# HKPolyU-UAV/FLVIS

Hardware: AMD Instinct MI355X
Metric: frames/sec/node (640×480 stereo+IMU) + ATE vs CPU ref, EuRoC MH_05 (higher is better)
Workload: dtype u8/f32 LK+GFTT, f64 geometry+BA

## Files before the change

flvis_amd/csrc/lk_kernel.hip:

```cpp
#include "dev_common.hpp"
#include "img_kernels.hpp"

namespace flvis {

constexpr int LK_WIN = 31;
constexpr int LK_PS = 40;
constexpr int LK_PROWS = 34;
constexpr int LK_RM = 4;
constexpr int LK_RS = 52;
constexpr int LK_RROWS = 33 + 2 * LK_RM;
constexpr int LK_TC_HDR = 64;
constexpr int LK_TC_LVL = 64 * 24;

typedef short lk_s2 __attribute__((ext_vector_type(2)));
typedef __attribute__((address_space(1))) uint32_t lk_gu32;
typedef uint32_t lk_u4 __attribute__((ext_vector_type(4)));
__device__ __forceinline__ lk_s2 lk_as_s2(uint32_t v) { return __builtin_bit_cast(lk_s2, v); }

__device__ __forceinline__ bool lk_load_patch(const uint8_t* __restrict__ img, int w, int h, int pitch, int bx, int by, int X0, int Y0,
                                              int nrows, uint8_t* patch) {
  if (X0 >= -bx && Y0 >= -by && X0 + 39 < w + bx && Y0 + nrows <= h + by) {
    const lk_gu32* const base = (const lk_gu32*)(img + (ptrdiff_t)Y0 * pitch + (X0 & ~3));
    const int sh = X0 & 3;
    int r = (int)threadIdx.x / 9, k = (int)threadIdx.x - 9 * r;
    unsigned off = (unsigned)(r * pitch + 4 * k);
    static_assert(LK_PROWS * 9 <= 5 * 64, "five trips");
    const int n = nrows * 9;
    uint32_t lo[5], hi[5];
#pragma unroll
    for (int t = 0; t < 5; t++) {
      const bool on = (int)threadIdx.x + 64 * t < n;
      const unsigned o = on ? off : 0u;
      lo[t] = *(const lk_gu32*)((const __attribute__((address_space(1))) uint8_t*)base + o);
      hi[t] = *(const lk_gu32*)((const __attribute__((address_space(1))) uint8_t*)base + o + 4);
      k += 1;
      const bool wrap = k >= 9;
      k = wrap ? k - 9 : k;
      off += (unsigned)(7 * pitch + 4) + (wrap ? (unsigned)(pitch - 36) : 0u);
    }
#pragma unroll
    for (int t = 0; t < 5; t++) asm volatile("" : "+v"(lo[t]), "+v"(hi[t]));
    r = (int)threadIdx.x / 9;
    k = (int)threadIdx.x - 9 * r;
    unsigned dst = (unsigned)(r * LK_PS + 4 * k);
#pragma unroll
    for (int t = 0; t < 5; t++) {
      if ((int)threadIdx.x + 64 * t < n) *reinterpret_cast<uint32_t*>(patch + dst) = __builtin_amdgcn_alignbyte(hi[t], lo[t], sh);
      k += 1;
      const bool wrap = k >= 9;
      k = wrap ? k - 9 : k;
      dst += (unsigned)(7 * LK_PS + 4) + (wrap ? (unsigned)(LK_PS - 36) : 0u);
    }
    return false;
  }
  for (int i = threadIdx.x; i < nrows * 9; i += 64) {
    int r = i / 9, k = i - r * 9;
    int Y = Y0 + r, X = X0 + 4 * k;
    uint32_t v;
    if (Y >= 0 && Y < h && X >= 0 && X + 3 < w) {
      const uint8_t* row = img + (size_t)Y * pitch;
      int a = X & ~3, sh = X & 3;
      uint32_t lo = *reinterpret_cast<const uint32_t*>(row + a);
      uint32_t hi = sh ? *reinterpret_cast<const uint32_t*>(row + a + 4) : 0u;
      v = __builtin_amdgcn_alignbyte(hi, lo, sh);
    } else {
      const uint8_t* row = img + (size_t)reflect101c(Y, h) * pitch;
      uint32_t b0 = row[reflect101c(X, w)], b1 = row[reflect101c(X + 1, w)], b2 = row[reflect101c(X + 2, w)],
               b3 = row[reflect101c(X + 3, w)];
      v = b0 | (b1 << 8) | (b2 << 16) | (b3 << 24);
    }
    *reinterpret_cast<uint32_t*>(patch + r * LK_PS + 4 * k) = v;
  }
  return true;
}

__device__ __forceinline__ bool lk_load_region(const uint8_t* __restrict__ img, int w, int h, int pitch, int bx, int by, int X0, int Y0,
                                               uint8_t* region) {
  if (X0 >= -bx && Y0 >= -by && X0 + 51 < w + bx && Y0 + LK_RROWS <= h + by) {
    const __attribute__((address_space(1))) uint8_t* const base = (const __attribute__((address_space(1))) uint8_t*)(img + (ptrdiff_t)Y0 * pitch + X0);
    int r = (int)threadIdx.x / 13, k = (int)threadIdx.x - 13 * r;
    unsigned off = (unsigned)(r * pitch + 4 * k);
    static_assert(LK_RS == 52, "the region rows are contiguous in LDS: item i sits at byte 4 i");
    constexpr int N = LK_RROWS * 13, T = (N + 63) / 64;
    uint32_t v[T];
#pragma unroll
    for (int t = 0; t < T; t++) {
      const bool on = 64 * (t + 1) <= N || (int)threadIdx.x + 64 * t < N;
      v[t] = *(const lk_gu32*)(base + (on ? off : 0u));
      k += 12;
      const bool wrap = k >= 13;
      k = wrap ? k - 13 : k;
      off += (unsigned)(4 * pitch + 48) + (wrap ? (unsigned)(pitch - 52) : 0u);
    }
#pragma unroll
    for (int t = 0; t < T; t++) asm volatile("" : "+v"(v[t]));
#pragma unroll
    for (int t = 0; t < T; t++)
      if (64 * (t + 1) <= N || (int)threadIdx.x + 64 * t < N) *reinterpret_cast<uint32_t*>(region + 4 * ((int)threadIdx.x + 64 * t)) = v[t];
    return false;
  }
  for (int i = threadIdx.x; i < LK_RROWS * 13; i += 64) {
    int r = i / 13, k = i - r * 13;
    int Y = Y0 + r, X = X0 + 4 * k;
    uint32_t v;
    if (Y >= 0 && Y < h && X >= 0 && X + 3 < w) {
      v = *reinterpret_cast<const uint32_t*>(img + (size_t)Y * pitch + X);
    } else {
      const uint8_t* row = img + (size_t)reflect101c(Y, h) * pitch;
      uint32_t b0 = row[reflect101c(X, w)], b1 = row[reflect101c(X + 1, w)], b2 = row[reflect101c(X + 2, w)],
               b3 = row[reflect101c(X + 3, w)];
      v = b0 | (b1 << 8) | (b2 << 16) | (b3 << 24);
    }
    *reinterpret_cast<uint32_t*>(region + r * LK_RS + 4 * k) = v;
  }
  return true;
}

#define LK_PAIR(D, K)                                                                                              \
  ((((K)&3) == 3) ? __builtin_amdgcn_perm((D)[((K) >> 2) + 1], (D)[(K) >> 2], 0x0c040c03u)                         \
                  : __builtin_amdgcn_perm(0u, (D)[(K) >> 2], 0x0c000c00u | (uint32_t)((K)&3) | ((uint32_t)(((K)&3) + 1) << 16)))

__device__ __forceinline__ int lk_dot2_bias(lk_s2 a, lk_s2 b, int bias_uniform) {
  int r;
  asm("v_dot2_i32_i16 %0, %1, %2, %3" : "=v"(r) : "v"(a), "v"(b), "s"(bias_uniform));
  return r;
}
__device__ __forceinline__ void lk_wave_sum2_f32(int v1, int v2, float& f1, float& f2) {
  int a = v1 & 0xffff, b = v1 >> 16, c = v2 & 0xffff, d = v2 >> 16;
#define LK_STEP4(CTRL, RM)                                           \
  {                                                                  \
    const int ta = __builtin_amdgcn_update_dpp(0, a, CTRL, RM, 0xf, false); \
    const int tb = __builtin_amdgcn_update_dpp(0, b, CTRL, RM, 0xf, false); \
    const int tc = __builtin_amdgcn_update_dpp(0, c, CTRL, RM, 0xf, false); \
    const int td = __builtin_amdgcn_update_dpp(0, d, CTRL, RM, 0xf, false); \
    a += ta, b += tb, c += tc, d += td;                              \
  }
  LK_STEP4(0xB1, 0xf)
  LK_STEP4(0x4E, 0xf)
  LK_STEP4(0x141, 0xf)
  LK_STEP4(0x140, 0xf)
  LK_STEP4(0x142, 0xa)
  LK_STEP4(0x143, 0xc)
#undef LK_STEP4
  const float g1 = (float)__builtin_fma((double)b, 65536.0, (double)a), g2 = (float)__builtin_fma((double)d, 65536.0, (double)c);
  f1 = __builtin_bit_cast(float, __builtin_amdgcn_readlane(__builtin_bit_cast(int, g1), 63));
  f2 = __builtin_bit_cast(float, __builtin_amdgcn_readlane(__builtin_bit_cast(int, g2), 63));
}

__device__ __forceinline__ void lk_wave_sum3_wide(int v1, int v2, int v3, long long& s1, long long& s2, long long& s3) {
  int a = v1 & 0xffff, b = v1 >> 16, c = v2 & 0xffff, d = v2 >> 16, e = v3 & 0xffff, f = v3 >> 16;
#define LK_STEP6(CTRL, RM)                                                    \
  {                                                                           \
    const int ta = __builtin_amdgcn_update_dpp(0, a, CTRL, RM, 0xf, false);  \
    const int tb = __builtin_amdgcn_update_dpp(0, b, CTRL, RM, 0xf, false);  \
    const int tc = __builtin_amdgcn_update_dpp(0, c, CTRL, RM, 0xf, false);  \
    const int td = __builtin_amdgcn_update_dpp(0, d, CTRL, RM, 0xf, false);  \
    const int te = __builtin_amdgcn_update_dpp(0, e, CTRL, RM, 0xf, false);  \
    const int tf = __builtin_amdgcn_update_dpp(0, f, CTRL, RM, 0xf, false);  \
    a += ta, b += tb, c += tc, d += td, e += te, f += tf;                     \
  }
  LK_STEP6(0xB1, 0xf)
  LK_STEP6(0x4E, 0xf)
  LK_STEP6(0x141, 0xf)
  LK_STEP6(0x140, 0xf)
  LK_STEP6(0x142, 0xa)
  LK_STEP6(0x143, 0xc)
#undef LK_STEP6
  s1 = ((long long)__builtin_amdgcn_readlane(b, 63) << 16) + (long long)__builtin_amdgcn_readlane(a, 63);
  s2 = ((long long)__builtin_amdgcn_readlane(d, 63) << 16) + (long long)__builtin_amdgcn_readlane(c, 63);
  s3 = ((long long)__builtin_amdgcn_readlane(f, 63) << 16) + (long long)__builtin_amdgcn_readlane(e, 63);
}

template <bool INTERIOR>
__device__ __forceinline__ void lk_template(const uint8_t* patch, int lane, int ipx, int ipy, int W, int H, lk_s2 wT, lk_s2 wB,
                                            lk_s2 (&tI)[8], lk_s2 (&tX)[8], lk_s2 (&tY)[8], int& a11, int& a12, int& a22) {
  constexpr int W_BITS = 14;
  const int r = lane >> 1, c0 = (lane & 1) * 16;
  uint32_t d[3][5];
#pragma unroll
  for (int j = 0; j < 3; j++)
#pragma unroll
    for (int k = 0; k < 5; k++) d[j][k] = *reinterpret_cast<const uint32_t*>(patch + (r + j) * LK_PS + c0 + 4 * k);
  uint32_t bits = 0;
  if (!INTERIOR) {
    const int xs = ipx + c0, Y = ipy + r;
    int lo = -xs, hi = W - xs;
    lo = lo < 0 ? 0 : (lo > 18 ? 18 : lo);
    hi = hi < 0 ? 0 : (hi > 18 ? 18 : hi);
    bits = (Y >= 0 && Y < H && hi > lo) ? (((1u << hi) - 1u) & ~((1u << lo) - 1u)) : 0u;
  }
  lk_s2 DX[2][9], DY[2][9];
  {
    lk_s2 T0[10], T1[10];
#pragma unroll
    for (int j = 0; j < 10; j++) {
      const lk_s2 A = __builtin_bit_cast(lk_s2, LK_PAIR(d[0], 2 * j)), B = __builtin_bit_cast(lk_s2, LK_PAIR(d[1], 2 * j)),
                  Cc = __builtin_bit_cast(lk_s2, LK_PAIR(d[2], 2 * j));
      T0[j] = (A + Cc) * (short)3 + B * (short)10;
      T1[j] = Cc - A;
    }
    const int up2 = ((lane + 2) & 63) * 4;
#pragma unroll
    for (int j = 0; j < 9; j++) {
      DX[0][j] = T0[j + 1] - T0[j];
      const lk_s2 T1o = __builtin_bit_cast(lk_s2, __builtin_amdgcn_perm(__builtin_bit_cast(uint32_t, T1[j + 1]),
                                                                       __builtin_bit_cast(uint32_t, T1[j]), 0x05040302u));
      DY[0][j] = (T1[j + 1] + T1[j]) * (short)3 + T1o * (short)10;
      if (!INTERIOR) {
        const uint32_t m = ((bits >> (2 * j)) & 1u ? 0x0000ffffu : 0u) | ((bits >> (2 * j + 1)) & 1u ? 0xffff0000u : 0u);
        DX[0][j] = __builtin_bit_cast(lk_s2, __builtin_bit_cast(uint32_t, DX[0][j]) & m);
        DY[0][j] = __builtin_bit_cast(lk_s2, __builtin_bit_cast(uint32_t, DY[0][j]) & m);
      }
      DX[1][j] = __builtin_bit_cast(lk_s2, __builtin_amdgcn_ds_bpermute(up2, __builtin_bit_cast(int, DX[0][j])));
      DY[1][j] = __builtin_bit_cast(lk_s2, __builtin_amdgcn_ds_bpermute(up2, __builtin_bit_cast(int, DY[0][j])));
    }
  }
  if (r < LK_WIN) {
#pragma unroll
    for (int c2 = 0; c2 < 8; c2++) {
      int iv[2], ix[2], iy[2];
#pragma unroll
      for (int hh = 0; hh < 2; hh++) {
        const int c = 2 * c2 + hh;
        lk_s2 x0, x1, y0, y1;
        if (hh == 0) {
          x0 = DX[0][c2]; x1 = DX[1][c2]; y0 = DY[0][c2]; y1 = DY[1][c2];
        } else {
          x0 = __builtin_bit_cast(lk_s2, __builtin_amdgcn_perm(__builtin_bit_cast(uint32_t, DX[0][c2 + 1]), __builtin_bit_cast(uint32_t, DX[0][c2]), 0x05040302u));
          x1 = __builtin_bit_cast(lk_s2, __builtin_amdgcn_perm(__builtin_bit_cast(uint32_t, DX[1][c2 + 1]), __builtin_bit_cast(uint32_t, DX[1][c2]), 0x05040302u));
          y0 = __builtin_bit_cast(lk_s2, __builtin_amdgcn_perm(__builtin_bit_cast(uint32_t, DY[0][c2 + 1]), __builtin_bit_cast(uint32_t, DY[0][c2]), 0x05040302u));
          y1 = __builtin_bit_cast(lk_s2, __builtin_amdgcn_perm(__builtin_bit_cast(uint32_t, DY[1][c2 + 1]), __builtin_bit_cast(uint32_t, DY[1][c2]), 0x05040302u));
        }
        int ax = lk_dot2_bias(x0, wT, 1 << (W_BITS - 1)), ay = lk_dot2_bias(y0, wT, 1 << (W_BITS - 1));
        int ai = lk_dot2_bias(__builtin_bit_cast(lk_s2, LK_PAIR(d[1], c + 1)), wT, 1 << (W_BITS - 5 - 1));
        ax = __builtin_amdgcn_sdot2(x1, wB, ax, false);
        ay = __builtin_amdgcn_sdot2(y1, wB, ay, false);
        ai = __builtin_amdgcn_sdot2(__builtin_bit_cast(lk_s2, LK_PAIR(d[2], c + 1)), wB, ai, false);
        const bool on = c0 + c < LK_WIN;
        ix[hh] = on ? (ax >> W_BITS) : 0;
        iy[hh] = on ? (ay >> W_BITS) : 0;
        iv[hh] = on ? (ai >> (W_BITS - 5)) : 0;
      }
      tI[c2] = __builtin_bit_cast(lk_s2, __builtin_amdgcn_perm((uint32_t)iv[1], (uint32_t)iv[0], 0x05040100u));
      tX[c2] = __builtin_bit_cast(lk_s2, __builtin_amdgcn_perm((uint32_t)ix[1], (uint32_t)ix[0], 0x05040100u));
      tY[c2] = __builtin_bit_cast(lk_s2, __builtin_amdgcn_perm((uint32_t)iy[1], (uint32_t)iy[0], 0x05040100u));
      a11 = __builtin_amdgcn_sdot2(tX[c2], tX[c2], a11, false);
      a12 = __builtin_amdgcn_sdot2(tX[c2], tY[c2], a12, false);
      a22 = __builtin_amdgcn_sdot2(tY[c2], tY[c2], a22, false);
    }
  } else {
#pragma unroll
    for (int c = 0; c < 8; c++) {
      tI[c] = lk_s2{0, 0};
      tX[c] = lk_s2{0, 0};
      tY[c] = lk_s2{0, 0};
    }
  }
}

__device__ __forceinline__ bool lk_template_level(const uint8_t* img, int W, int H, int pitch, int bx, int by, int ipx, int ipy, int iw00,
                                                  int iw01, int iw10, int iw11, uint8_t* patch, int lane, lk_s2 (&tI)[8], lk_s2 (&tX)[8],
                                                  lk_s2 (&tY)[8], long long& iA11, long long& iA12, long long& iA22) {
  __syncthreads();
  const bool slow = lk_load_patch(img, W, H, pitch, bx, by, ipx - 1, ipy - 1, LK_PROWS, patch);
  __syncthreads();
  int a11 = 0, a12 = 0, a22 = 0;
  const bool interior = ipx >= 0 && ipx + 32 <= W - 1 && ipy >= 0 && ipy + 31 <= H - 1;
  const lk_s2 wT = lk_s2{(short)iw00, (short)iw01}, wB = lk_s2{(short)iw10, (short)iw11};
  if (interior)
    lk_template<true>(patch, lane, ipx, ipy, W, H, wT, wB, tI, tX, tY, a11, a12, a22);
  else
    lk_template<false>(patch, lane, ipx, ipy, W, H, wT, wB, tI, tX, tY, a11, a12, a22);
  lk_wave_sum3_wide(a11, a12, a22, iA11, iA12, iA22);
  return slow;
}
struct LKTmpl {
  uint32_t w[24];
  long long a11, a12, a22;
};
__device__ __noinline__ void lk_template_level_cold(const uint8_t* img, int W, int H, int pitch, int bx, int by, int ipx, int ipy, int iw00,
                                                    int iw01, int iw10, int iw11, uint8_t* patch, int lane, LKTmpl* out) {
  lk_s2 tI[8], tX[8], tY[8];
  long long a11, a12, a22;
  lk_template_level(img, W, H, pitch, bx, by, ipx, ipy, iw00, iw01, iw10, iw11, patch, lane, tI, tX, tY, a11, a12, a22);
#pragma unroll
  for (int k = 0; k < 8; k++) {
    out->w[k] = __builtin_bit_cast(uint32_t, tI[k]);
    out->w[8 + k] = __builtin_bit_cast(uint32_t, tX[k]);
    out->w[16 + k] = __builtin_bit_cast(uint32_t, tY[k]);
  }
  out->a11 = a11;
  out->a12 = a12;
  out->a22 = a22;
}

__device__ __forceinline__ void lk_tc_store_level(uint32_t* tc_ptr, int level, int lane, const lk_s2 (&tI)[8], const lk_s2 (&tX)[8],
                                                  const lk_s2 (&tY)[8], long long iA11, long long iA12, long long iA22) {
  lk_u4* dst = reinterpret_cast<lk_u4*>(tc_ptr + LK_TC_HDR + (size_t)level * LK_TC_LVL) + lane;
  uint32_t wI[8];
#pragma unroll
  for (int k = 0; k < 8; k++) wI[k] = __builtin_bit_cast(uint32_t, tI[k]);
  if (lane == 63) {
    wI[0] = (uint32_t)iA11; wI[1] = (uint32_t)((unsigned long long)iA11 >> 32);
    wI[2] = (uint32_t)iA12; wI[3] = (uint32_t)((unsigned long long)iA12 >> 32);
    wI[4] = (uint32_t)iA22; wI[5] = (uint32_t)((unsigned long long)iA22 >> 32);
  }
#pragma unroll
  for (int k = 0; k < 2; k++) {
    __builtin_nontemporal_store(lk_u4{wI[4 * k], wI[4 * k + 1], wI[4 * k + 2], wI[4 * k + 3]}, dst + 64 * k);
    __builtin_nontemporal_store(lk_u4{__builtin_bit_cast(uint32_t, tX[4 * k]), __builtin_bit_cast(uint32_t, tX[4 * k + 1]),
                                      __builtin_bit_cast(uint32_t, tX[4 * k + 2]), __builtin_bit_cast(uint32_t, tX[4 * k + 3])}, dst + 64 * (2 + k));
    __builtin_nontemporal_store(lk_u4{__builtin_bit_cast(uint32_t, tY[4 * k]), __builtin_bit_cast(uint32_t, tY[4 * k + 1]),
                                      __builtin_bit_cast(uint32_t, tY[4 * k + 2]), __builtin_bit_cast(uint32_t, tY[4 * k + 3])}, dst + 64 * (4 + k));
  }
}

__device__ __forceinline__ const uint8_t* lk_level_ptr(const PyrSel& P, int level, int s, int kc, const uint8_t* ind0) {
  const ImgSel& I = P.lvl[level];
  if (I.ind) return (level == 0 ? ind0 : *I.ind) + (size_t)s * P.stride[level];
  return I.b[I.cur ? (kc ^ I.flip) : 0] + (size_t)s * P.stride[level];
}

#ifndef FLVIS_LK_WAVES
#define FLVIS_LK_WAVES 4
#endif
#ifndef FLVIS_LK_WAVES_T
#define FLVIS_LK_WAVES_T 4
#endif
#ifdef FLVIS_LK_UTIL
__device__ unsigned long long g_lk_wt[3][8][32768][2];
#define LK_UTIL_BEGIN const unsigned long long lk_t0_ = wall_clock64(); const unsigned lk_widx_ = (blockIdx.y * gridDim.x + blockIdx.x) & 32767u;
#define LK_UTIL_END(ROLE)                                                              \
  if (threadIdx.x == 0) {                                                              \
    unsigned long long* u_ = g_lk_wt[(ROLE) % 3][prm.dbg_slot & 7][lk_widx_];          \
    u_[0] = lk_t0_;                                                                    \
    u_[1] = wall_clock64();                                                            \
  }
#else
#define LK_UTIL_BEGIN
#define LK_UTIL_END(ROLE)
#endif
template <int ROLE>
__device__ __forceinline__ void lk_track_body(const PyrSel& prev, const PyrSel& next, const float* __restrict__ prev_pts,
                                              float* __restrict__ next_pts, uint8_t* __restrict__ status,
                                              const int* __restrict__ count, int nmax, const LKParams& prm,
                                              const int* __restrict__ active) {
  int s = blockIdx.y, bx = blockIdx.x;
  {
    const int G = gridDim.x, N = G * gridDim.y;
    if ((N & 7) == 0) {
      const int L = bx + G * s;
      const int Lp = (L & 7) * (N >> 3) + (L >> 3);
      s = Lp / G;
      bx = Lp - s * G;
    }
  }
  if (active && !active[s]) return;
  int n = count[s];
  if (n > nmax) n = nmax;
  if (bx >= n) return;
  LK_UTIL_BEGIN
  __shared__ __attribute__((aligned(16))) uint8_t patch[LK_RROWS * LK_RS + 12];
  const int lane = threadIdx.x;
  int kc_prev = 0, kc_next = 0;
#pragma unroll
  for (int l = LK_MAX_LEVELS - 1; l >= 0; l--) {
    if (l <= prev.levels && prev.lvl[l].cur) kc_prev = prev.lvl[l].cur[s];
    if (l <= next.levels && next.lvl[l].cur) kc_next = next.lvl[l].cur[s];
  }
  const uint8_t* const ind_prev0 = prev.lvl[0].ind ? *prev.lvl[0].ind : nullptr;
  const uint8_t* const ind_next0 = next.lvl[0].ind ? *next.lvl[0].ind : nullptr;
  const int r = lane >> 1;
  const int c0 = (lane & 1) * 16;
  const int W_BITS = 14;
  double eps2 = prm.eps2;
  if (ROLE == 1) asm volatile("" : "+v"(eps2));
  const float FLT_SCALE = 1.f / (1 << 20);
  const float halfWin = (LK_WIN - 1) * 0.5f;

  for (int pb = bx; pb < n; pb += gridDim.x) {
    const int p = prm.order == 1 ? n - 1 - pb : pb;
    const size_t pi = ((size_t)s * nmax + p) * 2;
    const float ppx0 = prev_pts[pi], ppy0 = prev_pts[pi + 1];
    float nx = next_pts[pi], ny = next_pts[pi + 1];
    int st = 1;
    uint32_t* tc_ptr = nullptr;
    bool tc_store = false, tc_hit = false;
    uint32_t tc_mask = 0;
    if (ROLE == 2 && prm.tc_mode == 1) {
      if (p < prm.tc_cap) {
        tc_store = true;
        tc_ptr = prm.tc + ((size_t)s * prm.tc_cap + p) * prm.tc_stride;
      }
    } else if (ROLE == 1 && prm.tc_mode == 2) {
      const int code = __builtin_amdgcn_readfirstlane(prm.tc_slot[(size_t)s * nmax + p]);
      if (code >= 0 && (code & 0xffff) < prm.tc_cap) {
        tc_ptr = prm.tc + ((size_t)s * prm.tc_cap + (code & 0xffff)) * prm.tc_stride;
        tc_hit = true;
        tc_mask = (uint32_t)code >> 16;
      }
    }
    lk_u4 pq[6] = {};
    int pq_level = -1;
    for (int level = prev.levels; level >= 0; level--) {
      const float sc = (float)(1. / (1 << level));
      float ppx = ppx0 * sc, ppy = ppy0 * sc;
      float npx, npy;
      if (level == prev.levels) {
        if (prm.use_initial) {
          npx = nx * sc;
          npy = ny * sc;
        } else {
          npx = ppx;
          npy = ppy;
        }
      } else {
        npx = nx * 2.f;
        npy = ny * 2.f;
      }
      nx = npx;
      ny = npy;
      const int W = prev.w[level], H = prev.h[level];
      ppx -= halfWin;
      ppy -= halfWin;
      const int ipx = (int)floorf(ppx), ipy = (int)floorf(ppy);
      if (ipx < -LK_WIN || ipx >= W || ipy < -LK_WIN || ipy >= H) {
        if (level == 0) st = 0;
        continue;
      }
      float a = ppx - (float)ipx, b = ppy - (float)ipy;
      int iw00 = __float2int_rn((1.f - a) * (1.f - b) * (float)(1 << W_BITS));
      int iw01 = __float2int_rn(a * (1.f - b) * (float)(1 << W_BITS));
      int iw10 = __float2int_rn((1.f - a) * b * (float)(1 << W_BITS));
      int iw11 = (1 << W_BITS) - iw00 - iw01 - iw10;

      lk_s2 tI[8], tX[8], tY[8];
      long long iA11, iA12, iA22;
      const bool cached = ROLE == 1 && tc_hit && ((tc_mask >> level) & 1u);
      constexpr bool kEarlyRegion = ROLE == 1;
      int JW = 0, JH = 0;
      const uint8_t* Jimg = nullptr;
      if (kEarlyRegion) {
        JW = next.w[level], JH = next.h[level];
        Jimg = lk_level_ptr(next, level, s, kc_next, ind_next0);
      }
      bool region_ok = false;
      int RX0 = 0, RY0 = 0;
      if (cached) {
        if (prm.stats_tc && lane == 0) atomicAdd(&prm.stats_tc[0], 1ull);
        if (pq_level != level) {
          const lk_u4* src = reinterpret_cast<const lk_u4*>(tc_ptr + LK_TC_HDR + (size_t)level * LK_TC_LVL) + lane;
#pragma unroll
          for (int k = 0; k < 6; k++) pq[k] = __builtin_nontemporal_load(src + 64 * k);
        }
        if (kEarlyRegion) {
        {
          const int einx = (int)floorf(npx - halfWin), einy = (int)floorf(npy - halfWin);
          if (!(einx < -LK_WIN || einx >= JW || einy < -LK_WIN || einy >= JH)) {
            RX0 = (einx - LK_RM) & ~3;
            RY0 = einy - LK_RM;
            __syncthreads();
            const bool slow = lk_load_region(Jimg, JW, JH, next.pitch[level], next.bx[level], next.by[level], RX0, RY0, patch);
            __syncthreads();
            if (prm.stats_tc && slow && lane == 0) atomicAdd(&prm.stats_tc[2], 1ull);
            region_ok = true;
          }
        }
        }
        lk_u4 q[6];
#pragma unroll
        for (int k = 0; k < 6; k++) q[k] = pq[k];
        pq_level = -1;
        iA11 = (long long)(((unsigned long long)(uint32_t)__builtin_amdgcn_readlane((int)q[0].y, 63) << 32) | (uint32_t)__builtin_amdgcn_readlane((int)q[0].x, 63));
        iA12 = (long long)(((unsigned long long)(uint32_t)__builtin_amdgcn_readlane((int)q[0].w, 63) << 32) | (uint32_t)__builtin_amdgcn_readlane((int)q[0].z, 63));
        iA22 = (long long)(((unsigned long long)(uint32_t)__builtin_amdgcn_readlane((int)q[1].y, 63) << 32) | (uint32_t)__builtin_amdgcn_readlane((int)q[1].x, 63));
#pragma unroll
        for (int k = 0; k < 2; k++) {
          tI[4 * k + 0] = lk_as_s2(q[k].x); tI[4 * k + 1] = lk_as_s2(q[k].y);
          tI[4 * k + 2] = lk_as_s2(q[k].z); tI[4 * k + 3] = lk_as_s2(q[k].w);
          tX[4 * k + 0] = lk_as_s2(q[2 + k].x); tX[4 * k + 1] = lk_as_s2(q[2 + k].y);
          tX[4 * k + 2] = lk_as_s2(q[2 + k].z); tX[4 * k + 3] = lk_as_s2(q[2 + k].w);
          tY[4 * k + 0] = lk_as_s2(q[4 + k].x); tY[4 * k + 1] = lk_as_s2(q[4 + k].y);
          tY[4 * k + 2] = lk_as_s2(q[4 + k].z); tY[4 * k + 3] = lk_as_s2(q[4 + k].w);
        }
      } else if (ROLE == 1) {
        LKTmpl T;
        lk_template_level_cold(lk_level_ptr(prev, level, s, kc_prev, ind_prev0), W, H, prev.pitch[level], prev.bx[level], prev.by[level], ipx, ipy, iw00,
                               iw01, iw10, iw11, patch, lane, &T);
#pragma unroll
        for (int k = 0; k < 8; k++) {
          tI[k] = lk_as_s2(T.w[k]);
          tX[k] = lk_as_s2(T.w[8 + k]);
          tY[k] = lk_as_s2(T.w[16 + k]);
        }
        iA11 = T.a11;
        iA12 = T.a12;
        iA22 = T.a22;
      } else {
        const bool slow = lk_template_level(lk_level_ptr(prev, level, s, kc_prev, ind_prev0), W, H, prev.pitch[level], prev.bx[level], prev.by[level], ipx,
                                            ipy, iw00, iw01, iw10, iw11, patch, lane, tI, tX, tY, iA11, iA12, iA22);
        if (prm.stats_tc && slow && lane == 0) atomicAdd(&prm.stats_tc[1], 1ull);
        if (ROLE == 2 && tc_store) {
          lk_tc_store_level(tc_ptr, level, lane, tI, tX, tY, iA11, iA12, iA22);
          tc_mask |= 1u << level;
        }
      }
      const float A11 = (float)iA11 * FLT_SCALE, A12 = (float)iA12 * FLT_SCALE, A22 = (float)iA22 * FLT_SCALE;
      float D = A11 * A22 - A12 * A12;
      const float minEig = __fdiv_rn(A22 + A11 - sqrtf((A11 - A22) * (A11 - A22) + 4.f * A12 * A12),
                                     (float)(2 * LK_WIN * LK_WIN));
      if (minEig < prm.min_eig || D < 1.1920929e-07f) {
        if (level == 0) st = 0;
        continue;
      }
      D = __fdiv_rn(1.f, D);
      npx -= halfWin;
      npy -= halfWin;
      float pdx = 0.f, pdy = 0.f;
      if (!kEarlyRegion) {
        JW = next.w[level], JH = next.h[level];
        Jimg = lk_level_ptr(next, level, s, kc_next, ind_next0);
      }
      int iters_run = 0;
      for (int j = 0; j < prm.max_iter; j++) {
        iters_run = j + 1;
        const int inx = (int)floorf(npx), iny = (int)floorf(npy);
        if (inx < -LK_WIN || inx >= JW || iny < -LK_WIN || iny >= JH) {
          if (level == 0) st = 0;
          break;
        }
        a = npx - (float)inx;
        b = npy - (float)iny;
        iw00 = __float2int_rn((1.f - a) * (1.f - b) * (float)(1 << W_BITS));
        iw01 = __float2int_rn(a * (1.f - b) * (float)(1 << W_BITS));
        iw10 = __float2int_rn((1.f - a) * b * (float)(1 << W_BITS));
        iw11 = (1 << W_BITS) - iw00 - iw01 - iw10;
        if (!region_ok || inx < RX0 || inx - RX0 > 15 || iny < RY0 || iny - RY0 > 2 * LK_RM) {
          RX0 = (inx - LK_RM) & ~3;
          RY0 = iny - LK_RM;
          __syncthreads();
          const bool slow = lk_load_region(Jimg, JW, JH, next.pitch[level], next.bx[level], next.by[level], RX0, RY0, patch);
          __syncthreads();
          if (prm.stats_tc && slow && lane == 0) atomicAdd(&prm.stats_tc[2], 1ull);
          region_ok = true;
        }
        int b1 = 0, b2 = 0;
        if (r < LK_WIN) {
          const int bx = inx - RX0 + c0, sh = bx & 3;
          const uint8_t* rp = patch + (iny - RY0 + r) * LK_RS + (bx & ~3);
          uint32_t e[2][5];
#pragma unroll
          for (int q = 0; q < 2; q++) {
            uint32_t dd[6];
#pragma unroll
            for (int k = 0; k < 6; k++) dd[k] = *reinterpret_cast<const uint32_t*>(rp + q * LK_RS + 4 * k);
#pragma unroll
            for (int k = 0; k < 5; k++) e[q][k] = __builtin_amdgcn_alignbyte(dd[k + 1], dd[k], sh);
          }
          const lk_s2 wT = lk_s2{(short)iw00, (short)iw01}, wB = lk_s2{(short)iw10, (short)iw11};
#pragma unroll
          for (int c2 = 0; c2 < 8; c2++) {
            int iv[2];
#pragma unroll
            for (int hh = 0; hh < 2; hh++) {
              const int c = 2 * c2 + hh;
              const uint32_t pt = LK_PAIR(e[0], c), pb = LK_PAIR(e[1], c);
              int acc = lk_dot2_bias(__builtin_bit_cast(lk_s2, pt), wT, 1 << (W_BITS - 5 - 1));
              acc = __builtin_amdgcn_sdot2(__builtin_bit_cast(lk_s2, pb), wB, acc, false);
              iv[hh] = acc >> (W_BITS - 5);
            }
            const lk_s2 ivp = __builtin_bit_cast(lk_s2, __builtin_amdgcn_perm((uint32_t)iv[1], (uint32_t)iv[0], 0x05040100u));
            const lk_s2 diff = ivp - tI[c2];
            b1 = __builtin_amdgcn_sdot2(diff, tX[c2], b1, false);
            b2 = __builtin_amdgcn_sdot2(diff, tY[c2], b2, false);
          }
        }
        float sb1, sb2;
        lk_wave_sum2_f32(b1, b2, sb1, sb2);
        const float fb1 = sb1 * FLT_SCALE, fb2 = sb2 * FLT_SCALE;
        const float ddx = (A12 * fb2 - A22 * fb1) * D;
        const float ddy = (A12 * fb1 - A11 * fb2) * D;
        npx += ddx;
        npy += ddy;
        nx = npx + halfWin;
        ny = npy + halfWin;
        if ((double)ddx * (double)ddx + (double)ddy * (double)ddy <= eps2) break;
        if (j > 0 && fabs((double)(ddx + pdx)) < 0.01 && fabs((double)(ddy + pdy)) < 0.01) {
          nx -= ddx * 0.5f;
          ny -= ddy * 0.5f;
          break;
        }
        pdx = ddx;
        pdy = ddy;
      }
      if (prm.stats && lane == 0) {
        atomicAdd(&prm.stats[2 * level], (unsigned long long)iters_run);
        atomicAdd(&prm.stats[2 * level + 1], 1ull);
      }
      if (st && level == 0) {
        const float fx = nx - halfWin, fy = ny - halfWin;
        const int inx = (int)floorf(fx), iny = (int)floorf(fy);
        if (inx < -LK_WIN || inx >= JW || iny < -LK_WIN || iny >= JH) st = 0;
      }
    }
    if (lane == 0) {
      next_pts[pi] = nx;
      next_pts[pi + 1] = ny;
      status[(size_t)s * nmax + p] = (uint8_t)st;
      if (ROLE == 2 && tc_store) {
        tc_ptr[0] = __float_as_uint(ppx0);
        tc_ptr[1] = __float_as_uint(ppy0);
        *reinterpret_cast<long long*>(tc_ptr + 2) = prm.tc_tag[s];
        tc_ptr[4] = tc_mask;
      }
    }
  }
  LK_UTIL_END(ROLE)
}

__global__ __launch_bounds__(64) __attribute__((amdgpu_waves_per_eu(FLVIS_LK_WAVES, FLVIS_LK_WAVES))) void k_lk_track(
    PyrSel prev, PyrSel next, const float* __restrict__ prev_pts, float* __restrict__ next_pts, uint8_t* __restrict__ status,
    const int* __restrict__ count, int nmax, LKParams prm, const int* __restrict__ active) {
  lk_track_body<0>(prev, next, prev_pts, next_pts, status, count, nmax, prm, active);
}
__global__ __launch_bounds__(64) __attribute__((amdgpu_waves_per_eu(FLVIS_LK_WAVES_T, FLVIS_LK_WAVES_T))) void k_lk_track_temporal(
    PyrSel prev, PyrSel next, const float* __restrict__ prev_pts, float* __restrict__ next_pts, uint8_t* __restrict__ status,
    const int* __restrict__ count, int nmax, LKParams prm, const int* __restrict__ active) {
  lk_track_body<1>(prev, next, prev_pts, next_pts, status, count, nmax, prm, active);
}
__global__ __launch_bounds__(64) __attribute__((amdgpu_waves_per_eu(FLVIS_LK_WAVES, FLVIS_LK_WAVES))) void k_lk_track_stereo(
    PyrSel prev, PyrSel next, const float* __restrict__ prev_pts, float* __restrict__ next_pts, uint8_t* __restrict__ status,
    const int* __restrict__ count, int nmax, LKParams prm, const int* __restrict__ active) {
  lk_track_body<2>(prev, next, prev_pts, next_pts, status, count, nmax, prm, active);
}

int lk_tc_slot_dwords(int levels) { return LK_TC_HDR + (levels + 1) * LK_TC_LVL; }

void launch_lk_track(hipStream_t st, const PyrSel& prev, const PyrSel& next, const float* prev_pts, float* next_pts,
                     uint8_t* status, const int* count, int nmax, int S, LKParams prm, const int* active, int max_pts, int role) {
  int gx = nmax < 512 ? nmax : 512;
  if (max_pts > 0 && max_pts < gx) gx = (max_pts + 7) & ~7;
  if (gx > nmax) gx = nmax;
  if (role == 1)
    hipLaunchKernelGGL(k_lk_track_temporal, dim3(gx, S), dim3(64), 0, st, prev, next, prev_pts, next_pts, status, count, nmax, prm, active);
  else if (role == 2)
    hipLaunchKernelGGL(k_lk_track_stereo, dim3(gx, S), dim3(64), 0, st, prev, next, prev_pts, next_pts, status, count, nmax, prm, active);
  else
    hipLaunchKernelGGL(k_lk_track, dim3(gx, S), dim3(64), 0, st, prev, next, prev_pts, next_pts, status, count, nmax, prm, active);
}

}

#ifdef FLVIS_LK_UTIL
extern "C" int flvis_debug_lk_util(unsigned long long* out, int reset) {
  const size_t bytes = sizeof(unsigned long long) * 3 * 8 * 32768 * 2;
  if (out && hipMemcpyFromSymbol(out, HIP_SYMBOL(flvis::g_lk_wt), bytes) != hipSuccess) return -1;
  if (reset) {
    void* dp = nullptr;
    if (hipGetSymbolAddress(&dp, HIP_SYMBOL(flvis::g_lk_wt)) != hipSuccess || hipMemset(dp, 0, bytes) != hipSuccess) return -1;
  }
  return 0;
}
#endif
```

Before: 63130.

## Prefetch LK search region via global_load_lds DMA while building template

For non-ROLE-1 kernels the search region in the next image is given its own LDS buffer. Its load is issued asynchronously with global_load_lds before the template patch is built, so the fetch overlaps template construction instead of happening on the first iteration. The template-level block barriers become wave-level barriers for this path, and a vmcnt(0) wait follows. This costs extra LDS per block, which may reduce occupancy, and adds alignment and bounds preconditions for the DMA path.

```diff
diff --git a/flvis_amd/csrc/lk_kernel.hip b/flvis_amd/csrc/lk_kernel.hip
--- a/flvis_amd/csrc/lk_kernel.hip
+++ b/flvis_amd/csrc/lk_kernel.hip
@@ -17,19 +17,26 @@
 typedef uint32_t lk_u4 __attribute__((ext_vector_type(4)));
 __device__ __forceinline__ lk_s2 lk_as_s2(uint32_t v) { return __builtin_bit_cast(lk_s2, v); }
 
+__device__ __forceinline__ int lk_stage_lane() {
+  int t = (int)threadIdx.x;
+  asm volatile("" : "+v"(t));
+  return t;
+}
+
 __device__ __forceinline__ bool lk_load_patch(const uint8_t* __restrict__ img, int w, int h, int pitch, int bx, int by, int X0, int Y0,
                                               int nrows, uint8_t* patch) {
   if (X0 >= -bx && Y0 >= -by && X0 + 39 < w + bx && Y0 + nrows <= h + by) {
     const lk_gu32* const base = (const lk_gu32*)(img + (ptrdiff_t)Y0 * pitch + (X0 & ~3));
     const int sh = X0 & 3;
-    int r = (int)threadIdx.x / 9, k = (int)threadIdx.x - 9 * r;
+    const int tid = lk_stage_lane();
+    int r = tid / 9, k = tid - 9 * r;
     unsigned off = (unsigned)(r * pitch + 4 * k);
     static_assert(LK_PROWS * 9 <= 5 * 64, "five trips");
     const int n = nrows * 9;
     uint32_t lo[5], hi[5];
 #pragma unroll
     for (int t = 0; t < 5; t++) {
-      const bool on = (int)threadIdx.x + 64 * t < n;
+      const bool on = tid + 64 * t < n;
       const unsigned o = on ? off : 0u;
       lo[t] = *(const lk_gu32*)((const __attribute__((address_space(1))) uint8_t*)base + o);
       hi[t] = *(const lk_gu32*)((const __attribute__((address_space(1))) uint8_t*)base + o + 4);
@@ -40,12 +47,12 @@
     }
 #pragma unroll
     for (int t = 0; t < 5; t++) asm volatile("" : "+v"(lo[t]), "+v"(hi[t]));
-    r = (int)threadIdx.x / 9;
-    k = (int)threadIdx.x - 9 * r;
+    r = tid / 9;
+    k = tid - 9 * r;
     unsigned dst = (unsigned)(r * LK_PS + 4 * k);
 #pragma unroll
     for (int t = 0; t < 5; t++) {
-      if ((int)threadIdx.x + 64 * t < n) *reinterpret_cast<uint32_t*>(patch + dst) = __builtin_amdgcn_alignbyte(hi[t], lo[t], sh);
+      if (tid + 64 * t < n) *reinterpret_cast<uint32_t*>(patch + dst) = __builtin_amdgcn_alignbyte(hi[t], lo[t], sh);
       k += 1;
       const bool wrap = k >= 9;
       k = wrap ? k - 9 : k;
@@ -74,9 +81,13 @@
   return true;
 }
 
+__device__ __forceinline__ bool lk_region_inside(int w, int h, int bx, int by, int X0, int Y0) {
+  return X0 >= -bx && Y0 >= -by && X0 + 51 < w + bx && Y0 + LK_RROWS <= h + by;
+}
+
 __device__ __forceinline__ bool lk_load_region(const uint8_t* __restrict__ img, int w, int h, int pitch, int bx, int by, int X0, int Y0,
                                                uint8_t* region) {
-  if (X0 >= -bx && Y0 >= -by && X0 + 51 < w + bx && Y0 + LK_RROWS <= h + by) {
+  if (lk_region_inside(w, h, bx, by, X0, Y0)) {
     const __attribute__((address_space(1))) uint8_t* const base = (const __attribute__((address_space(1))) uint8_t*)(img + (ptrdiff_t)Y0 * pitch + X0);
     int r = (int)threadIdx.x / 13, k = (int)threadIdx.x - 13 * r;
     unsigned off = (unsigned)(r * pitch + 4 * k);
@@ -116,6 +127,34 @@
   return true;
 }
 
+constexpr int LK_RBUF = 9 * 256;
+static_assert(LK_RROWS * LK_RS <= LK_RBUF && (LK_RROWS * 13 + 63) / 64 == 9, "nine trips of 64 dwords hold the region");
+
+typedef __attribute__((address_space(3))) uint8_t lk_lds_u8;
+__device__ __forceinline__ void lk_issue_region(const uint8_t* __restrict__ img, int pitch, int X0, int Y0, lk_lds_u8* region) {
+  const __attribute__((address_space(1))) uint8_t* const base = (const __attribute__((address_space(1))) uint8_t*)(img + (ptrdiff_t)Y0 * pitch + X0);
+  const int tid = lk_stage_lane();
+  int r = tid / 13, k = tid - 13 * r;
+  unsigned off = (unsigned)(r * pitch + 4 * k);
+  constexpr int N = LK_RROWS * 13, T = (N + 63) / 64;
+#pragma unroll
+  for (int t = 0; t < T; t++) {
+    const bool on = 64 * (t + 1) <= N || tid + 64 * t < N;
+    __builtin_amdgcn_global_load_lds((const __attribute__((address_space(1))) void*)(base + (on ? off : 0u)),
+                                     (__attribute__((address_space(3))) void*)(region + 256 * t), 4, 0, 0);
+    k += 12;
+    const bool wrap = k >= 13;
+    k = wrap ? k - 13 : k;
+    off += (unsigned)(4 * pitch + 48) + (wrap ? (unsigned)(pitch - 52) : 0u);
+  }
+}
+
+__device__ __forceinline__ void lk_wave_sync() {
+  __builtin_amdgcn_fence(__ATOMIC_RELEASE, "wavefront");
+  __builtin_amdgcn_wave_barrier();
+  __builtin_amdgcn_fence(__ATOMIC_ACQUIRE, "wavefront");
+}
+
 #define LK_PAIR(D, K)                                                                                              \
   ((((K)&3) == 3) ? __builtin_amdgcn_perm((D)[((K) >> 2) + 1], (D)[(K) >> 2], 0x0c040c03u)                         \
                   : __builtin_amdgcn_perm(0u, (D)[(K) >> 2], 0x0c000c00u | (uint32_t)((K)&3) | ((uint32_t)(((K)&3) + 1) << 16)))
@@ -258,12 +297,13 @@
   }
 }
 
+template <bool DMA_BESIDE>
 __device__ __forceinline__ bool lk_template_level(const uint8_t* img, int W, int H, int pitch, int bx, int by, int ipx, int ipy, int iw00,
                                                   int iw01, int iw10, int iw11, uint8_t* patch, int lane, lk_s2 (&tI)[8], lk_s2 (&tX)[8],
                                                   lk_s2 (&tY)[8], long long& iA11, long long& iA12, long long& iA22) {
-  __syncthreads();
+  if (DMA_BESIDE) lk_wave_sync(); else __syncthreads();
   const bool slow = lk_load_patch(img, W, H, pitch, bx, by, ipx - 1, ipy - 1, LK_PROWS, patch);
-  __syncthreads();
+  if (DMA_BESIDE) lk_wave_sync(); else __syncthreads();
   int a11 = 0, a12 = 0, a22 = 0;
   const bool interior = ipx >= 0 && ipx + 32 <= W - 1 && ipy >= 0 && ipy + 31 <= H - 1;
   const lk_s2 wT = lk_s2{(short)iw00, (short)iw01}, wB = lk_s2{(short)iw10, (short)iw11};
@@ -282,7 +322,7 @@
                                                     int iw01, int iw10, int iw11, uint8_t* patch, int lane, LKTmpl* out) {
   lk_s2 tI[8], tX[8], tY[8];
   long long a11, a12, a22;
-  lk_template_level(img, W, H, pitch, bx, by, ipx, ipy, iw00, iw01, iw10, iw11, patch, lane, tI, tX, tY, a11, a12, a22);
+  lk_template_level<false>(img, W, H, pitch, bx, by, ipx, ipy, iw00, iw01, iw10, iw11, patch, lane, tI, tX, tY, a11, a12, a22);
 #pragma unroll
   for (int k = 0; k < 8; k++) {
     out->w[k] = __builtin_bit_cast(uint32_t, tI[k]);
@@ -360,7 +400,10 @@
   if (n > nmax) n = nmax;
   if (bx >= n) return;
   LK_UTIL_BEGIN
-  __shared__ __attribute__((aligned(16))) uint8_t patch[LK_RROWS * LK_RS + 12];
+  constexpr bool kRegionBeside = ROLE != 1;
+  __shared__ __attribute__((aligned(16))) uint8_t patch[kRegionBeside ? LK_PROWS * LK_PS : LK_RROWS * LK_RS + 12];
+  __shared__ __attribute__((aligned(kRegionBeside ? 256 : 16))) uint8_t region_buf[kRegionBeside ? LK_RBUF : 16];
+  uint8_t* const region = kRegionBeside ? region_buf : patch;
   const int lane = threadIdx.x;
   int kc_prev = 0, kc_next = 0;
 #pragma unroll
@@ -374,7 +417,7 @@
   const int c0 = (lane & 1) * 16;
   const int W_BITS = 14;
   double eps2 = prm.eps2;
-  if (ROLE == 1) asm volatile("" : "+v"(eps2));
+  if (ROLE == 1) asm volatile("" : "+v"(eps2)); else asm volatile("" : "+s"(eps2));
   const float FLT_SCALE = 1.f / (1 << 20);
   const float halfWin = (LK_WIN - 1) * 0.5f;
 
@@ -438,12 +481,8 @@
       long long iA11, iA12, iA22;
       const bool cached = ROLE == 1 && tc_hit && ((tc_mask >> level) & 1u);
       constexpr bool kEarlyRegion = ROLE == 1;
-      int JW = 0, JH = 0;
-      const uint8_t* Jimg = nullptr;
-      if (kEarlyRegion) {
-        JW = next.w[level], JH = next.h[level];
-        Jimg = lk_level_ptr(next, level, s, kc_next, ind_next0);
-      }
+      const int JW = next.w[level], JH = next.h[level];
+      const uint8_t* const Jimg = lk_level_ptr(next, level, s, kc_next, ind_next0);
       bool region_ok = false;
       int RX0 = 0, RY0 = 0;
       if (cached) {
@@ -497,8 +536,22 @@
         iA12 = T.a12;
         iA22 = T.a22;
       } else {
-        const bool slow = lk_template_level(lk_level_ptr(prev, level, s, kc_prev, ind_prev0), W, H, prev.pitch[level], prev.bx[level], prev.by[level], ipx,
-                                            ipy, iw00, iw01, iw10, iw11, patch, lane, tI, tX, tY, iA11, iA12, iA22);
+        const uint8_t* const Iimg = lk_level_ptr(prev, level, s, kc_prev, ind_prev0);
+        if (kRegionBeside) {
+          const int einx = (int)floorf(npx - halfWin), einy = (int)floorf(npy - halfWin);
+          const int ex0 = (einx - LK_RM) & ~3, ey0 = einy - LK_RM;
+          if (!(einx < -LK_WIN || einx >= JW || einy < -LK_WIN || einy >= JH) &&
+              lk_region_inside(JW, JH, next.bx[level], next.by[level], ex0, ey0) &&
+              (((uintptr_t)Jimg | (uintptr_t)next.pitch[level]) & 3) == 0) {
+            RX0 = ex0;
+            RY0 = ey0;
+            lk_issue_region(Jimg, next.pitch[level], RX0, RY0, (lk_lds_u8*)region_buf);
+            region_ok = true;
+          }
+        }
+        const bool slow = lk_template_level<kRegionBeside>(Iimg, W, H, prev.pitch[level], prev.bx[level],
+                                                           prev.by[level], ipx, ipy, iw00, iw01, iw10, iw11, patch, lane, tI, tX, tY, iA11, iA12, iA22);
+        if (kRegionBeside) asm volatile("s_waitcnt vmcnt(0)" ::: "memory");
         if (prm.stats_tc && slow && lane == 0) atomicAdd(&prm.stats_tc[1], 1ull);
         if (ROLE == 2 && tc_store) {
           lk_tc_store_level(tc_ptr, level, lane, tI, tX, tY, iA11, iA12, iA22);
@@ -517,10 +570,6 @@
       npx -= halfWin;
       npy -= halfWin;
       float pdx = 0.f, pdy = 0.f;
-      if (!kEarlyRegion) {
-        JW = next.w[level], JH = next.h[level];
-        Jimg = lk_level_ptr(next, level, s, kc_next, ind_next0);
-      }
       int iters_run = 0;
       for (int j = 0; j < prm.max_iter; j++) {
         iters_run = j + 1;
@@ -539,7 +588,7 @@
           RX0 = (inx - LK_RM) & ~3;
           RY0 = iny - LK_RM;
           __syncthreads();
-          const bool slow = lk_load_region(Jimg, JW, JH, next.pitch[level], next.bx[level], next.by[level], RX0, RY0, patch);
+          const bool slow = lk_load_region(Jimg, JW, JH, next.pitch[level], next.bx[level], next.by[level], RX0, RY0, region);
           __syncthreads();
           if (prm.stats_tc && slow && lane == 0) atomicAdd(&prm.stats_tc[2], 1ull);
           region_ok = true;
@@ -547,7 +596,7 @@
         int b1 = 0, b2 = 0;
         if (r < LK_WIN) {
           const int bx = inx - RX0 + c0, sh = bx & 3;
-          const uint8_t* rp = patch + (iny - RY0 + r) * LK_RS + (bx & ~3);
+          const uint8_t* rp = region + (iny - RY0 + r) * LK_RS + (bx & ~3);
           uint32_t e[2][5];
 #pragma unroll
           for (int q = 0; q < 2; q++) {
```

Result: no change. 63470 (median of 6 runs) (+0.5%).
